# ultralytics/yolov3

Hardware: NVIDIA H100
Metric: images/sec @640 bs32 YOLOv3 (higher is better)
Workload: dtype bf16

## Files before the change

yolov3_b200/csrc/y3_common.cuh:

```cuda
#pragma once
#include <utility>

#include <cuda.h>
#include <cuda_bf16.h>
#include <cuda_fp16.h>
#include <cuda_runtime.h>
#include <stdint.h>

namespace y3 {

#ifndef Y3_WATCHDOG_CYCLES
#define Y3_WATCHDOG_CYCLES 3000000000LL
#endif

__device__ __forceinline__ uint32_t smem_u32(const void* p) {
  return static_cast<uint32_t>(__cvta_generic_to_shared(p));
}

__device__ __forceinline__ void mbar_init(uint64_t* bar, uint32_t count) {
  asm volatile("mbarrier.init.shared::cta.b64 [%0], %1;" ::"r"(smem_u32(bar)), "r"(count) : "memory");
}
__device__ __forceinline__ void fence_mbar_init() {
  asm volatile("fence.mbarrier_init.release.cluster;" ::: "memory");
}
// ... 25 lines not shown
  while (!mbar_try_wait(bar, parity)) {
    if (clock64() - t0 > Y3_WATCHDOG_CYCLES) {
      if (err) atomicExch(err, code);
      __threadfence_system();
      __trap();
    }
  }
}

__device__ __forceinline__ void tma_prefetch_desc(const CUtensorMap* m) {
  asm volatile("prefetch.tensormap [%0];" ::"l"(reinterpret_cast<uint64_t>(m)) : "memory");
}
__device__ __forceinline__ void tma_load_2d(void* dst, const CUtensorMap* m, uint64_t* bar, int c0, int c1) {
  asm volatile(
      "cp.async.bulk.tensor.2d.shared::cluster.global.mbarrier::complete_tx::bytes [%0], [%1, {%3, %4}], [%2];"
      ::"r"(smem_u32(dst)), "l"(reinterpret_cast<uint64_t>(m)), "r"(smem_u32(bar)), "r"(c0), "r"(c1)
      : "memory");
}
__device__ __forceinline__ void tma_load_4d(void* dst, const CUtensorMap* m, uint64_t* bar, int c0, int c1, int c2, int c3) {
  asm volatile(
      "cp.async.bulk.tensor.4d.shared::cluster.global.mbarrier::complete_tx::bytes [%0], [%1, {%3, %4, %5, %6}], [%2];"
      ::"r"(smem_u32(dst)), "l"(reinterpret_cast<uint64_t>(m)), "r"(smem_u32(bar)), "r"(c0), "r"(c1), "r"(c2), "r"(c3)
      : "memory");
}
__device__ __forceinline__ void tma_load_5d(void* dst, const CUtensorMap* m, uint64_t* bar, int c0, int c1, int c2,
                                            int c3, int c4) {
  asm volatile(
      "cp.async.bulk.tensor.5d.shared::cluster.global.mbarrier::complete_tx::bytes [%0], [%1, {%3, %4, %5, %6, %7}], "
      "[%2];"
      ::"r"(smem_u32(dst)), "l"(reinterpret_cast<uint64_t>(m)), "r"(smem_u32(bar)), "r"(c0), "r"(c1), "r"(c2), "r"(c3),
      "r"(c4)
      : "memory");
}

__device__ __forceinline__ void tma_store_2d(const CUtensorMap* m, const void* src, int c0, int c1) {
  asm volatile("cp.async.bulk.tensor.2d.global.shared::cta.bulk_group [%0, {%2, %3}], [%1];" ::"l"(
                   reinterpret_cast<uint64_t>(m)),
               "r"(smem_u32(src)), "r"(c0), "r"(c1)
               : "memory");
}
__device__ __forceinline__ void tma_store_4d(const CUtensorMap* m, const void* src, int c0, int c1, int c2, int c3) {
  asm volatile("cp.async.bulk.tensor.4d.global.shared::cta.bulk_group [%0, {%2, %3, %4, %5}], [%1];" ::"l"(
                   reinterpret_cast<uint64_t>(m)),
               "r"(smem_u32(src)), "r"(c0), "r"(c1), "r"(c2), "r"(c3)
               : "memory");
}
__device__ __forceinline__ void bulk_commit_group() { asm volatile("cp.async.bulk.commit_group;" ::: "memory"); }
__device__ __forceinline__ void bulk_wait_read_all() { asm volatile("cp.async.bulk.wait_group.read 0;" ::: "memory"); }
__device__ __forceinline__ void bulk_wait_read_1() { asm volatile("cp.async.bulk.wait_group.read 1;" ::: "memory"); }
__device__ __forceinline__ void bulk_wait_all() { asm volatile("cp.async.bulk.wait_group 0;" ::: "memory"); }
__device__ __forceinline__ void named_bar_sync(int id, int nthreads) {
  asm volatile("bar.sync %0, %1;" ::"r"(id), "r"(nthreads) : "memory");
}
__device__ __forceinline__ uint4 lds128(uint32_t saddr) {
  uint4 v;
  asm volatile("ld.shared.v4.u32 {%0, %1, %2, %3}, [%4];" : "=r"(v.x), "=r"(v.y), "=r"(v.z), "=r"(v.w) : "r"(saddr));
  return v;
}
__device__ __forceinline__ void sts128(uint32_t saddr, uint4 v) {
  asm volatile("st.shared.v4.u32 [%0], {%1, %2, %3, %4};" ::"r"(saddr), "r"(v.x), "r"(v.y), "r"(v.z), "r"(v.w) : "memory");
}

__device__ __forceinline__ bool elect_one() {
  uint32_t pred;
  asm volatile(
      "{\n"
      ".reg .pred p;\n"
      "elect.sync _|p, 0xffffffff;\n"
      "selp.u32 %0, 1, 0, p;\n"
      "}\n"
      : "=r"(pred));
  return pred != 0;
}

__host__ __device__ constexpr uint32_t wgmma_layout(uint32_t swizzle_bytes) {
  return swizzle_bytes == 128 ? 1u : (swizzle_bytes == 64 ? 2u : 3u);
}
__host__ __device__ constexpr uint32_t wgmma_desc_hi(uint32_t sbo_bytes, uint32_t swizzle_bytes) {
  return ((sbo_bytes >> 4) & 0x3FFFu) | (wgmma_layout(swizzle_bytes) << 30);
}
__device__ __forceinline__ uint64_t wgmma_desc(uint32_t desc_hi, uint32_t saddr, uint32_t lbo_bytes = 0) {
  return (uint64_t(desc_hi) << 32) | ((saddr >> 4) & 0x3FFFu) | (((lbo_bytes >> 4) & 0x3FFFu) << 16);
}
__device__ __forceinline__ void wgmma_fence() { asm volatile("wgmma.fence.sync.aligned;" ::: "memory"); }
__device__ __forceinline__ void wgmma_commit() { asm volatile("wgmma.commit_group.sync.aligned;" ::: "memory"); }
// ... 279 lines not shown
```

yolov3_b200/csrc/y3_conv_tc.cu:

```cuda
#include <cuda_bf16.h>

#include <type_traits>

#include "y3_common.cuh"
#include "y3_internal.h"

namespace y3 {

namespace {

constexpr int kBlockM = 128;
constexpr int kThreads = 320;
constexpr int kProducerWarp = 8;
constexpr int kStoreWarp = 9;
constexpr int kSmemBudget = 221 * 1024;

template <int BLOCK_N, int BLOCK_K, bool HALO, int STAGE_ES = 2, bool STAGE_DQ = false>
struct Cfg {
  static constexpr uint32_t kARows = HALO ? kBlockM + 2 : kBlockM;
  static constexpr uint32_t kATxBytes = kARows * BLOCK_K * 2;
  static constexpr uint32_t kABytes = (kATxBytes + 1023u) / 1024u * 1024u;
  static constexpr uint32_t kTaps = HALO ? 3 : 1;
  static constexpr uint32_t kBBytes = BLOCK_N * BLOCK_K * 2;
  static constexpr uint32_t kStageBytes = kABytes + kTaps * kBBytes;
  static constexpr int kMaxStages = 8;
  static constexpr uint32_t kBarBytes = 256;
  static constexpr bool kStaged = BLOCK_N == 256 && STAGE_ES > 0;
  static constexpr uint32_t kTileBytes = kBlockM * BLOCK_N * (STAGE_ES > 0 ? STAGE_ES : 2);
  static constexpr uint32_t kOutBytes = kTileBytes + BLOCK_N * 4 * (STAGE_DQ ? 2 : 1);
  static constexpr bool kPair = BLOCK_N <= 128 && STAGE_ES > 0;
  static constexpr uint32_t kRowBytes = BLOCK_N * (STAGE_ES > 0 ? STAGE_ES : 2);
  static constexpr uint32_t kBoxBytes = kRowBytes < 128 ? kRowBytes : 128;
  static constexpr uint32_t kBoxes = kRowBytes / kBoxBytes;
  static constexpr uint32_t kPairBytes = 1024 - kBarBytes + 2 * kTileBytes;
  __host__ __device__ static constexpr int ring_stages(uint32_t reserve) {
    const int s = int(kSmemBudget - reserve) / int(kStageBytes);
    return s > kMaxStages ? kMaxStages : s;
  }
  __host__ __device__ static constexpr uint32_t bres_bytes(int steps) { return (uint32_t(steps) * kBBytes + 1023u) / 1024u * 1024u; }
  __host__ __device__ static constexpr int bres_stages(int steps, uint32_t reserve) {
    const int s = (int(kSmemBudget - reserve) - int(bres_bytes(steps))) / int(kABytes);
    return s > kMaxStages ? kMaxStages : s;
  }
  static constexpr uint32_t kSwizzleBytes = BLOCK_K * 2;
  static constexpr uint32_t kSbo = 8 * kSwizzleBytes;
  __host__ __device__ static constexpr uint32_t bar_offset(int stages, bool bres, int b_steps) {
    return uint32_t(stages) * kABytes + (bres ? bres_bytes(b_steps) : uint32_t(stages) * kTaps * kBBytes);
  }
  __host__ __device__ static constexpr uint32_t smem_end(int stages, bool bres, int b_steps, uint32_t reserve) {
    return bar_offset(stages, bres, b_steps) + kBarBytes + reserve;
  }
  static constexpr size_t kSmemBytes = size_t(kSmemBudget) + 1024  + kBarBytes;
  static_assert(ring_stages(kStaged ? kOutBytes : (kPair ? kPairBytes : 0u)) >= 2, "pipeline needs at least two stages");
  static_assert(!HALO || BLOCK_K >= 32, "halo reuse: rows of 64 or 128 bytes");
};

__device__ __forceinline__ float bias_act(float a, float b, bool silu) {
  if (!silu) return a + b;
  const float h = fmaf(a, 0.5f, b);
  float t;
  asm("tanh.approx.f32 %0, %1;" : "=f"(t) : "f"(h));
  return fmaf(h, t, h);
}

__device__ __forceinline__ float bias_act_dq(float a, float s, float b, bool silu) {
  const float h = fmaf(a, s, b);
  if (!silu) return h;
  float t;
  asm("tanh.approx.f32 %0, %1;" : "=f"(t) : "f"(h));
  return fmaf(h, t, h);
}

__device__ __forceinline__ void cp_async16(uint32_t saddr, const void* gptr) {
  asm volatile("cp.async.cg.shared.global [%0], [%1], 16;" ::"r"(saddr), "l"(gptr) : "memory");
}
__device__ __forceinline__ void cp_async_wait_all() { asm volatile("cp.async.wait_all;" ::: "memory"); }

__device__ __forceinline__ uint32_t fast_div(uint32_t n, uint32_t mul, uint32_t shr) {
  const uint32_t t = __umulhi(n, mul);
  return (t + ((n - t) >> (shr ? 1 : 0))) >> (shr ? shr - 1 : 0);
}

struct RowOut {
  __nv_bfloat16* out;
  float* f32;
  const __nv_bfloat16* res;
};

template <int ES, typename T>
__device__ __forceinline__ T* elem_ptr(T* p, long long off) {
  if (ES == 2) return p + off;
  return reinterpret_cast<T*>(reinterpret_cast<uintptr_t>(p) + off * ES);
}

template <int ES = 2>
__device__ __forceinline__ RowOut row_out(const ConvTcArgs& p, int mt, int n0, int m) {
  RowOut o{nullptr, nullptr, nullptr};
  bool valid;
  int img, oy, ox;
  if (p.mode == 0) {
    const int row = mt * kBlockM + m;
    const int plane = p.hp * p.wp;
    img = static_cast<int>(fast_div(static_cast<uint32_t>(row), p.plane_mul, p.plane_shr));
    const int rem = row - img * plane;
    const int yp = static_cast<int>(fast_div(static_cast<uint32_t>(rem), p.wp_mul, p.wp_shr)), xp = rem - yp * p.wp;
    valid = row < p.rows_total && yp >= 1 && yp <= p.hp - 2 && xp >= 1 && xp <= p.wp - 2;
    oy = yp - 1;
    ox = xp - 1;
  } else {
// ... 17 lines not shown
  } else if (p.upsample) {
    const long long r00 = (static_cast<long long>(img) * (2 * oh + 2) + 2 * oy + 1) * (2 * ow + 2) + 2 * ox + 1;
    o.out = elem_ptr<ES>(p.out, r00 * p.out_ld + p.out_coff + n0);
  } else {
    o.out = elem_ptr<ES>(p.out, conv_row * p.out_ld + p.out_coff + n0);
  }
  return o;
}

template <int BLOCK_N, int BLOCK_K, bool HALO, int IN_FMT = Y3_FMT_BF16, int OUT_FMT = Y3_FMT_BF16>
__global__ void __launch_bounds__(kThreads, 1)
conv_tc_kernel(const __grid_constant__ CUtensorMap map_a, const __grid_constant__ CUtensorMap map_b,
               const __grid_constant__ CUtensorMap map_out, const __grid_constant__ CUtensorMap map_res, const ConvTcArgs p) {
  constexpr bool kInE4m3 = IN_FMT == Y3_FMT_E4M3, kOutE4m3 = OUT_FMT == Y3_FMT_E4M3;
  using C = Cfg<BLOCK_N, BLOCK_K, HALO, kOutE4m3 ? 1 : (kInE4m3 ? 0 : 2), kInE4m3 && kOutE4m3>;
  constexpr int kOes = kOutE4m3 ? 1 : 2;
  constexpr int kKch = kInE4m3 ? 2 * BLOCK_K : BLOCK_K;
  using Mma = std::conditional_t<kInE4m3, WgmmaE4m3<BLOCK_N>, Wgmma<BLOCK_N>>;
  const int STAGES = p.stages;
  const bool bres = p.bres != 0;
  constexpr uint32_t kBStage = C::kTaps * C::kBBytes;
  const int b_steps = p.taps * p.kblocks;

  extern __shared__ uint8_t smem_raw[];
  const uint32_t raw_addr = smem_u32(smem_raw);
  uint8_t* smem = smem_raw + ((1024u - (raw_addr & 1023u)) & 1023u);
  uint8_t* smem_a = smem;
  uint8_t* smem_b = smem + STAGES * C::kABytes;
  uint64_t* full_bar = reinterpret_cast<uint64_t*>(smem_b + (bres ? C::bres_bytes(b_steps) : uint32_t(STAGES) * kBStage));
  uint64_t* empty_bar = full_bar + C::kMaxStages;
  uint64_t* bres_bar = empty_bar + C::kMaxStages;
  uint64_t* staged_bar = bres_bar + 1;
  uint64_t* done_bar = bres_bar + 3;
  uint32_t* stile = reinterpret_cast<uint32_t*>(reinterpret_cast<uint8_t*>(full_bar) + C::kBarBytes);
  float* sbias = reinterpret_cast<float*>(stile + C::kTileBytes / 4);
  float* sdq = sbias + BLOCK_N;
  const bool staged_out = C::kStaged && p.out_f32 == nullptr;
  uint8_t* ptile = reinterpret_cast<uint8_t*>(full_bar) + 1024;
  const bool pair_out = C::kPair && p.tile_tma != 0;

  const int warp = threadIdx.x >> 5;
  const int lane = threadIdx.x & 31;

  if (threadIdx.x == 0) {
    tma_prefetch_desc(&map_a);
    tma_prefetch_desc(&map_b);
    if (pair_out) {
      tma_prefetch_desc(&map_out);
      if (p.res) tma_prefetch_desc(&map_res);
    }
    for (int i = 0; i < STAGES; ++i) {
      mbar_init(&full_bar[i], 1);
      mbar_init(&empty_bar[i], 8);
    }
    mbar_init(bres_bar, 1);
    for (int b = 0; b < 2; ++b) {
      mbar_init(&staged_bar[b], pair_out ? 1 : 32);
      mbar_init(&done_bar[b], 8);
    }
    fence_mbar_init();
  }
  __syncthreads();
  pdl_wait();
  pdl_trigger();

  const int total_tiles = p.m_tiles * p.n_tiles;
  const int k_iters = HALO ? 3 * p.kblocks : p.taps * p.kblocks;

  if (warp == kProducerWarp) {
    uint32_t stage = 0, phase = 0;
    if (bres && int(blockIdx.x) < total_tiles && elect_one()) {
      mbar_expect_tx(bres_bar, uint32_t(b_steps) * C::kBBytes);
      for (int st = 0; st < b_steps; ++st) {
        const int kb = st / p.taps, tap = st - kb * p.taps;
        tma_load_2d(smem_b + st * C::kBBytes, &map_b, bres_bar, (p.custom_taps ? p.tap_wcol[tap] : tap) * p.cin + kb * kKch, 0);
      }
    }
    __syncwarp();
    const int n_tiles = p.n_tiles, wp = p.wp, cin = p.cin, a_coff = p.a_coff, a_ld = p.a_ld;
    const int taps_it = HALO ? 3 : p.taps;
    const bool xpair = p.xpair != 0, nine = p.taps == 9, custom = p.custom_taps != 0;
    const int taps_w = xpair ? 2 : 3;
    const uint32_t stage_tx = p.a_tx_bytes + (bres ? 0u : kBStage);
    auto run = [&](auto mode_tag) {
      constexpr int MODE = decltype(mode_tag)::value;
      for (int tile = blockIdx.x; tile < total_tiles; tile += gridDim.x) {
        const int nt = tile % n_tiles;
        const int mt = tile / n_tiles;
        const int n0 = nt * BLOCK_N;
        int row0 = 0, img = 0, oh0 = 0, ow0 = 0;
// ... 21 lines not shown
            if (MODE == 0)
              tma_load_2d(a_dst, &map_a, &full_bar[stage], a_coff + kcol, row0 + shift);
            else
              tma_load_5d(a_dst, &map_a, &full_bar[stage], c0, ow0 + c1, r & 1, oh0 + (r >> 1), img);
            if (!bres) {
#pragma unroll
              for (uint32_t t = 0; t < C::kTaps; ++t)
                tma_load_2d(b_dst + t * C::kBBytes, &map_b, &full_bar[stage], bcol + int(t) * cin, n0);
            }
          }
          __syncwarp();
          if (++stage == uint32_t(STAGES)) {
            stage = 0;
            phase ^= 1u;
          }
          if (++s == taps_w) {
            s = 0;
            ++r;
          }
          if (++tap == taps_it) {
            tap = 0;
            r = 0;
            s = 0;
            ++kb;
          }
        }
      }
    };
    if (p.mode == 0)
      run(std::integral_constant<int, 0>{});
    else
      run(std::integral_constant<int, 1>{});
  } else if (warp == kStoreWarp) {
    if (pair_out) {
      if (lane != 0) return;
      const uint32_t res_tx = uint32_t(p.mode == 0 ? kBlockM : p.tw * p.th) * C::kRowBytes;
      constexpr int kBoxCh = C::kBoxBytes / kOes;
      auto move = [&](int tile, int b, bool load) {
        const int mt = tile / p.n_tiles, n0 = (tile % p.n_tiles) * BLOCK_N;
        int c1 = mt * kBlockM, c2 = 0, c3 = 0;
        if (p.mode != 0) {
          const int per_img = p.tiles_w * p.tiles_h;
          c3 = mt / per_img;
          const int t = mt - c3 * per_img;
          c1 = (t % p.tiles_w) * p.tw;
          c2 = (t / p.tiles_w) * p.th;
        }
#pragma unroll
        for (uint32_t k = 0; k < C::kBoxes; ++k) {
          uint8_t* s = ptile + b * C::kTileBytes + k * kBlockM * C::kBoxBytes;
          const int c0 = (load ? p.res_coff : p.out_coff) + n0 + int(k) * kBoxCh;
          if (load) {
            if (p.mode == 0) tma_load_2d(s, &map_res, &staged_bar[b], c0, c1);
            else tma_load_4d(s, &map_res, &staged_bar[b], c0, c1, c2, c3);
          } else {
            if (p.mode == 0) tma_store_2d(&map_out, s, c0, c1);
            else tma_store_4d(&map_out, s, c0, c1, c2, c3);
          }
        }
      };
      auto stage = [&](int tile, int b) {
        if (p.res) {
          mbar_expect_tx(&staged_bar[b], res_tx);
          move(tile, b, true);
        } else {
          mbar_arrive(&staged_bar[b]);
        }
      };
      const int step = int(gridDim.x);
      if (int(blockIdx.x) < total_tiles) stage(blockIdx.x, 0);
      if (int(blockIdx.x) + step < total_tiles) stage(blockIdx.x + step, 1);
      for (int tile = blockIdx.x, i = 0; tile < total_tiles; tile += step, ++i) {
        const int b = i & 1;
        mbar_wait(&done_bar[b], uint32_t(i >> 1) & 1u, p.err, 9);
        move(tile, b, false);
        bulk_commit_group();
        if (tile + 2 * step < total_tiles) {
          bulk_wait_read_all();
          stage(tile + 2 * step, b);
        }
      }
      bulk_wait_all();
      return;
    }
    if (!staged_out) return;
    const int r = lane & 7, c = lane >> 3;
    const uint32_t stile_s = smem_u32(stile);
    struct Rows {
      __nv_bfloat16* out[4];
      const __nv_bfloat16* res[4];
    };
    auto rows_of = [&](int tile, Rows& R) {
      const int mt = tile / p.n_tiles, n0 = (tile % p.n_tiles) * BLOCK_N;
#pragma unroll
      for (int q = 0; q < 4; ++q) {
        const RowOut ro = row_out<kOes>(p, mt, n0, 32 * q + lane);
        R.out[q] = ro.out;
        R.res[q] = ro.res;
      }
    };
    constexpr int kCh = 16 / kOes, kRowChunks = BLOCK_N / kCh;
    auto chunk = [&](int h, int w, int j) { return uint32_t((h * kRowChunks + j) * 64 + w * 8 + r); };
    auto src_lane = [&](int h, int w) { return (w & 1) * 16 + 8 * h + r; };
    auto stage_bias = [&](int tile) {
      const int n0 = (tile % p.n_tiles) * BLOCK_N;
      for (int i = lane; i < BLOCK_N / 4; i += 32)
        if (n0 + 4 * i < p.cout) {
          cp_async16(smem_u32(sbias + 4 * i), p.bias + n0 + 4 * i);
          if (kInE4m3) cp_async16(smem_u32(sdq + 4 * i), p.dq + n0 + 4 * i);
        }
    };
    auto stage_res = [&](int tile, const Rows& R) {
      const int n0 = (tile % p.n_tiles) * BLOCK_N;
      if (p.res) {
#pragma unroll
        for (int h = 0; h < 2; ++h)
#pragma unroll
          for (int w = 0; w < 8; ++w) {
            const auto* res = reinterpret_cast<const __nv_bfloat16*>(
                __shfl_sync(~0u, reinterpret_cast<unsigned long long>(R.res[2 * (w >> 2) + ((w & 3) >> 1)]), src_lane(h, w)));
            if (!res) continue;
#pragma unroll 1
            for (int jg = 0; jg < kRowChunks / 4; ++jg) {
              const int j = 4 * jg + c;
              if (kOutE4m3 ? n0 + kCh * j < p.cout : n0 + 32 * jg < p.cout)
                cp_async16(stile_s + 16u * chunk(h, w, j), elem_ptr<kOes>(res, kCh * j));
            }
          }
      }
      cp_async_wait_all();
      mbar_arrive(staged_bar);
    };
    auto drain = [&](int tile, const Rows& R) {
      const int n0 = (tile % p.n_tiles) * BLOCK_N;
      const long long up_row_stride = static_cast<long long>(2 * (p.mode == 0 ? p.wp - 2 : p.wo) + 2) * p.out_ld;
      const int reps = p.upsample ? 4 : 1;
      const uint4* tile16 = reinterpret_cast<const uint4*>(stile);
#pragma unroll
      for (int h = 0; h < 2; ++h)
#pragma unroll
        for (int w = 0; w < 8; ++w) {
          auto* out = reinterpret_cast<__nv_bfloat16*>(
              __shfl_sync(~0u, reinterpret_cast<unsigned long long>(R.out[2 * (w >> 2) + ((w & 3) >> 1)]), src_lane(h, w)));
          if (!out) continue;
#pragma unroll 2
          for (int jg = 0; jg < kRowChunks / 4; ++jg) {
            const int j = 4 * jg + c;
            if (kOutE4m3 ? n0 + kCh * j >= p.cout : n0 + 32 * jg >= p.cout) break;
            const uint4 v = tile16[chunk(h, w, j)];
            for (int rep = 0; rep < reps; ++rep)
              *reinterpret_cast<uint4*>(elem_ptr<kOes>(out, (rep >> 1) * up_row_stride + (rep & 1) * p.out_ld + kCh * j)) = v;
          }
        }
    };
    uint32_t tphase = 0;
    Rows cur, nxt;
    if (int(blockIdx.x) < total_tiles) {
      rows_of(blockIdx.x, cur);
      stage_bias(blockIdx.x);
      stage_res(blockIdx.x, cur);
    }
    for (int tile = blockIdx.x; tile < total_tiles; tile += gridDim.x) {
      const int next = tile + int(gridDim.x);
      if (next < total_tiles) rows_of(next, nxt);
      mbar_wait(done_bar, tphase, p.err, 7);
      tphase ^= 1u;
      if (next < total_tiles) stage_bias(next);
      drain(tile, cur);
      if (next < total_tiles) stage_res(next, nxt);
      cur = nxt;
    }
  } else {
    const int wg = warp >> 2;
    const int m0 = wg * 64 + (warp & 3) * 16 + (lane >> 2);
    const int cq = 2 * (lane & 3);
    constexpr uint32_t kDescHi = wgmma_desc_hi(C::kSbo, C::kSwizzleBytes);
    const uint32_t a_base = smem_u32(smem_a) + uint32_t(wg) * 64u * C::kSwizzleBytes;
    const uint32_t b_base = smem_u32(smem_b);
    uint32_t stage = 0, phase = 0, tphase = 0;
    if (bres && int(blockIdx.x) < total_tiles) mbar_wait(bres_bar, 0, p.err, 6);
    for (int tile = blockIdx.x, ti = 0; tile < total_tiles; tile += gridDim.x, ++ti) {
      float acc[BLOCK_N / 2];
      uint32_t prev = 0;
      for (int it = 0; it < k_iters; ++it) {
        mbar_wait(&full_bar[stage], phase, p.err, 3);
        const uint32_t a_st = a_base + stage * C::kABytes;
        const uint32_t b_st = b_base + (bres ? uint32_t(it) : stage) * kBStage;
        wgmma_fence();
#pragma unroll
        for (uint32_t t = 0; t < C::kTaps; ++t) {
#pragma unroll
          for (int k = 0; k < BLOCK_K / 16; ++k) {
            const uint64_t adesc = wgmma_desc(kDescHi, a_st + t * C::kSwizzleBytes + k * 32);
            const uint64_t bdesc = wgmma_desc(kDescHi, b_st + t * C::kBBytes + k * 32);
            Mma::template mma<0, 0>(acc, adesc, bdesc, (it != 0 || t != 0 || k != 0) ? 1u : 0u);
          }
        }
        wgmma_commit();
        wgmma_wait<1>();
        if (it > 0 && lane == 0) mbar_arrive(&empty_bar[prev]);
        prev = stage;
        if (++stage == uint32_t(STAGES)) {
          stage = 0;
          phase ^= 1u;
        }
      }
      wgmma_wait<0>();
      wgmma_fence_regs(acc);
      if (lane == 0) mbar_arrive(&empty_bar[prev]);

      const bool silu = p.act == Y3_ACT_SILU;
      const float bscale = silu ? 0.5f : 1.0f;
      if (staged_out) {
        mbar_wait(staged_bar, tphase, p.err, 8);
        tphase ^= 1u;
        const bool has_res = p.res != nullptr;
        if constexpr (kOutE4m3) {
          uint8_t* tb = reinterpret_cast<uint8_t*>(stile) + ((warp * 8 + (lane >> 2)) * 16 + cq);
#pragma unroll
          for (int j = 0; j < BLOCK_N / 8; ++j) {
            const float2 b = *reinterpret_cast<const float2*>(sbias + 8 * j + cq);
            float2 q = b;
            if (kInE4m3) q = *reinterpret_cast<const float2*>(sdq + 8 * j + cq);
#pragma unroll
            for (int h = 0; h < 2; ++h) {
              uint16_t& hw = *reinterpret_cast<uint16_t*>(tb + (h * BLOCK_N / 16 + j / 2) * 64 * 16 + (j & 1) * 8);
              float x0, x1;
              if (kInE4m3) {
                x0 = bias_act_dq(acc[4 * j + 2 * h], bscale * q.x, bscale * b.x, silu);
                x1 = bias_act_dq(acc[4 * j + 2 * h + 1], bscale * q.y, bscale * b.y, silu);
              } else {
                x0 = bias_act(acc[4 * j + 2 * h], bscale * b.x, silu);
                x1 = bias_act(acc[4 * j + 2 * h + 1], bscale * b.y, silu);
              }
              if (has_res) {
                const float2 f = unpack_e4m3x2(hw);
                x0 = fmaf(p.res_scale, f.x, x0);
                x1 = fmaf(p.res_scale, f.y, x1);
              }
              hw = pack_e4m3x2(x0 * p.out_inv_scale, x1 * p.out_inv_scale);
            }
          }
          __syncwarp();
          if (lane == 0) mbar_arrive(done_bar);
          continue;
        }
        uint32_t* words = stile + threadIdx.x;
#pragma unroll
        for (int j = 0; j < BLOCK_N / 8; ++j) {
          const float2 b = *reinterpret_cast<const float2*>(sbias + 8 * j + cq);
#pragma unroll
          for (int h = 0; h < 2; ++h) {
            uint32_t& word = words[(h * BLOCK_N / 8 + j) * 256];
            float x0 = bias_act(acc[4 * j + 2 * h], bscale * b.x, silu);
            float x1 = bias_act(acc[4 * j + 2 * h + 1], bscale * b.y, silu);
            if (has_res) {
              const float2 f = unpack_bf16x2(word);
              x0 += f.x;
              x1 += f.y;
            }
            word = pack_bf16x2(x0, x1);
          }
        }
        __syncwarp();
        if (lane == 0) mbar_arrive(done_bar);
      } else if (pair_out) {
        const int b = ti & 1;
        mbar_wait(&staged_bar[b], uint32_t(ti >> 1) & 1u, p.err, 10);
        uint8_t* tb = ptile + b * C::kTileBytes;
        const int n0 = (tile % p.n_tiles) * BLOCK_N;
        const bool has_res = p.res != nullptr;
        uint32_t rowoff[2], sw[2];
        bool valid[2];
#pragma unroll
        for (int h = 0; h < 2; ++h) {
          const int m = m0 + 8 * h;
          rowoff[h] = uint32_t(m) * C::kBoxBytes;
          sw[h] = ((rowoff[h] >> 7) & (C::kBoxBytes / 16 - 1)) << 4;
          valid[h] = true;
          if (p.mode == 0) {
            const int row = (tile / p.n_tiles) * kBlockM + m;
            const int img = static_cast<int>(fast_div(static_cast<uint32_t>(row), p.plane_mul, p.plane_shr));
            const int rem = row - img * (p.hp * p.wp);
            const int yp = static_cast<int>(fast_div(static_cast<uint32_t>(rem), p.wp_mul, p.wp_shr)), xp = rem - yp * p.wp;
            valid[h] = yp >= 1 && yp <= p.hp - 2 && xp >= 1 && xp <= p.wp - 2;
          }
        }
#pragma unroll
        for (int j = 0; j < BLOCK_N / 8; ++j) {
          const int c = 8 * j + cq;
          const bool in = n0 + c < p.cout;
          const float2 bv = in ? __ldg(reinterpret_cast<const float2*>(p.bias + n0 + c)) : make_float2(0.f, 0.f);
          float2 qv = bv;
          if (kInE4m3) qv = in ? __ldg(reinterpret_cast<const float2*>(p.dq + n0 + c)) : make_float2(0.f, 0.f);
          const uint32_t xb = uint32_t(8 * j * kOes);
          const uint32_t region = xb / C::kBoxBytes * (kBlockM * C::kBoxBytes), xin = xb % C::kBoxBytes;
#pragma unroll
          for (int h = 0; h < 2; ++h) {
            uint8_t* pp = tb + region + rowoff[h] + (xin ^ sw[h]) + cq * kOes;
            float x0, x1;
            if (kInE4m3) {
              x0 = bias_act_dq(acc[4 * j + 2 * h], bscale * qv.x, bscale * bv.x, silu);
              x1 = bias_act_dq(acc[4 * j + 2 * h + 1], bscale * qv.y, bscale * bv.y, silu);
            } else {
              x0 = bias_act(acc[4 * j + 2 * h], bscale * bv.x, silu);
              x1 = bias_act(acc[4 * j + 2 * h + 1], bscale * bv.y, silu);
            }
            if constexpr (kOutE4m3) {
              uint16_t& hw = *reinterpret_cast<uint16_t*>(pp);
              if (has_res) {
                const float2 f = unpack_e4m3x2(hw);
                x0 = fmaf(p.res_scale, f.x, x0);
                x1 = fmaf(p.res_scale, f.y, x1);
              }
              hw = valid[h] ? pack_e4m3x2(x0 * p.out_inv_scale, x1 * p.out_inv_scale) : uint16_t(0);
            } else {
              uint32_t& word = *reinterpret_cast<uint32_t*>(pp);
              if (has_res) {
                const float2 f = unpack_bf16x2(word);
                x0 += f.x;
                x1 += f.y;
              }
              word = valid[h] ? pack_bf16x2(x0, x1) : 0u;
            }
          }
        }
        fence_proxy_async_smem();
        __syncwarp();
        if (lane == 0) mbar_arrive(&done_bar[b]);
      } else {
        const int mt = tile / p.n_tiles, n0 = (tile % p.n_tiles) * BLOCK_N;
        const long long up_row_stride = static_cast<long long>(2 * (p.mode == 0 ? p.wp - 2 : p.wo) + 2) * p.out_ld;
        const int reps = p.upsample ? 4 : 1;
        constexpr int kChunk = BLOCK_N == 256 ? 1 : (kInE4m3 && BLOCK_N == 128 ? 8 : (BLOCK_N / 8 < 16 ? BLOCK_N / 8 : 16));
#pragma unroll
        for (int h = 0; h < 2; ++h) {
          const RowOut ro = row_out<kOes>(p, mt, n0, m0 + 8 * h);
          if (!ro.f32 && !ro.out) continue;
#pragma unroll
          for (int j0 = 0; j0 < BLOCK_N / 8; j0 += kChunk) {
            float2 b[kChunk], q[kChunk];
            uint32_t r[kChunk];
#pragma unroll
            for (int jj = 0; jj < kChunk; ++jj) {
              const int c = 8 * (j0 + jj) + cq;
              const bool in = p.out_f32 || n0 + c < p.cout;
              b[jj] = in ? __ldg(reinterpret_cast<const float2*>(p.bias + n0 + c)) : make_float2(0.f, 0.f);
              if (kInE4m3) q[jj] = in ? __ldg(reinterpret_cast<const float2*>(p.dq + n0 + c)) : make_float2(0.f, 0.f);
              if (kOutE4m3)
                r[jj] = (in && ro.res) ? __ldcg(reinterpret_cast<const unsigned short*>(elem_ptr<1>(ro.res, c))) : 0u;
              else
                r[jj] = (in && ro.res) ? __ldcg(reinterpret_cast<const unsigned int*>(ro.res + c)) : 0u;
            }
#pragma unroll
            for (int jj = 0; jj < kChunk; ++jj) {
              const int c = 8 * (j0 + jj) + cq;
              if (!p.out_f32 && n0 + c >= p.cout) continue;
              float x0, x1;
              if (kInE4m3) {
                x0 = bias_act_dq(acc[4 * (j0 + jj) + 2 * h], bscale * q[jj].x, bscale * b[jj].x, silu);
                x1 = bias_act_dq(acc[4 * (j0 + jj) + 2 * h + 1], bscale * q[jj].y, bscale * b[jj].y, silu);
              } else {
                x0 = bias_act(acc[4 * (j0 + jj) + 2 * h], bscale * b[jj].x, silu);
                x1 = bias_act(acc[4 * (j0 + jj) + 2 * h + 1], bscale * b[jj].y, silu);
              }
              if (ro.f32) {
                *reinterpret_cast<float2*>(ro.f32 + c) = make_float2(x0, x1);
              } else if (kOutE4m3) {
                if (ro.res) {
                  const float2 f = unpack_e4m3x2(static_cast<uint16_t>(r[jj]));
                  x0 = fmaf(p.res_scale, f.x, x0);
// ... 1 lines not shown
                }
                const uint16_t v = pack_e4m3x2(x0 * p.out_inv_scale, x1 * p.out_inv_scale);
                for (int rep = 0; rep < reps; ++rep)
                  *reinterpret_cast<uint16_t*>(elem_ptr<1>(ro.out, (rep >> 1) * up_row_stride + (rep & 1) * p.out_ld + c)) = v;
              } else {
                if (ro.res) {
                  const float2 f = unpack_bf16x2(r[jj]);
                  x0 += f.x;
                  x1 += f.y;
                }
                const uint32_t v = pack_bf16x2(x0, x1);
                for (int rep = 0; rep < reps; ++rep)
                  *reinterpret_cast<uint32_t*>(ro.out + (rep >> 1) * up_row_stride + (rep & 1) * p.out_ld + c) = v;
              }
            }
          }
        }
      }
    }
  }
}

template <int BLOCK_N, int BLOCK_K, bool HALO = false, int IN_FMT = Y3_FMT_BF16, int OUT_FMT = Y3_FMT_BF16>
int launch_cfg(const ConvTcPlan& plan, cudaStream_t stream) {
  constexpr bool kInE4m3 = IN_FMT == Y3_FMT_E4M3, kOutE4m3 = OUT_FMT == Y3_FMT_E4M3;
  using C = Cfg<BLOCK_N, BLOCK_K, HALO, kOutE4m3 ? 1 : (kInE4m3 ? 0 : 2), kInE4m3 && kOutE4m3>;
  auto kern = conv_tc_kernel<BLOCK_N, BLOCK_K, HALO, IN_FMT, OUT_FMT>;
  static bool attr_set = false;
  if (!attr_set) {
    Y3_CHECK_CUDA(cudaFuncSetAttribute(kern, cudaFuncAttributeMaxDynamicSharedMemorySize, int(C::kSmemBytes)));
    attr_set = true;
  }
  ConvTcArgs args = plan.args;
  const bool out_tile = C::kStaged && args.out_f32 == nullptr;
  const bool pair = C::kPair && args.tile_tma != 0;
  const uint32_t reserve = out_tile ? C::kOutBytes : (pair ? C::kPairBytes : 0u);
  const int b_steps = args.taps * args.kblocks;
  args.bres = plan.bres;
  args.stages = plan.bres ? C::bres_stages(b_steps, reserve) : C::ring_stages(reserve);
  if (args.bres && args.stages < 3) {
    args.bres = 0;
    args.stages = C::ring_stages(reserve);
  }
  if (args.stages < 2 || args.stages > C::kMaxStages ||
      C::smem_end(args.stages, args.bres != 0, b_steps, reserve) + 1024u > C::kSmemBytes)
    return set_error(Y3_ERR_BAD_ARG, "conv_tc: %d ring stages (resident weights %d, output tiles %u bytes) do not fit %zu bytes of shared memory (N=%d K=%d)",
                     args.stages, args.bres, reserve, C::kSmemBytes, BLOCK_N, BLOCK_K);
  Y3_CHECK_CUDA(launch_pdl(kern, dim3(plan.grid), dim3(kThreads), C::kSmemBytes, stream, plan.map_a, plan.map_b,
                           plan.map_out, plan.map_res, args));
  return Y3_OK;
}

int pick_block_n(int cout) { return cout <= 32 ? 32 : (cout <= 64 ? 64 : (cout <= 128 ? 128 : 256)); }

template <int IN_FMT, int OUT_FMT>
int launch_fmt(const ConvTcPlan& plan, cudaStream_t stream) {
#define Y3_DISPATCH_K(BN)                                                        \
  switch (plan.block_k) {                                                        \
    case 64: return launch_cfg<BN, 64, false, IN_FMT, OUT_FMT>(plan, stream);    \
    case 32: return launch_cfg<BN, 32, false, IN_FMT, OUT_FMT>(plan, stream);    \
    case 16: return launch_cfg<BN, 16, false, IN_FMT, OUT_FMT>(plan, stream);    \
  }                                                                              \
  break;
  constexpr bool kHalo = !(IN_FMT == Y3_FMT_E4M3 && OUT_FMT == Y3_FMT_BF16);
  if (plan.halo) {
    if constexpr (kHalo) {
      if (plan.block_k == 64) {
        if (plan.block_n == 128) return launch_cfg<128, 64, true, IN_FMT, OUT_FMT>(plan, stream);
        if (plan.block_n == 64) return launch_cfg<64, 64, true, IN_FMT, OUT_FMT>(plan, stream);
// ... 177 lines not shown
      const int thc = th > a.ho ? a.ho : th;
      const long long tiles = static_cast<long long>((a.wo + tw - 1) / tw) * ((a.ho + thc - 1) / thc);
      if (best_tiles < 0 || tiles < best_tiles || (tiles == best_tiles && tw > best_tw)) {
        best_tiles = tiles;
        best_tw = tw;
        best_th = thc;
      }
    }
    a.tw = best_tw;
    a.th = best_th;
    a.tiles_w = (a.wo + a.tw - 1) / a.tw;
    a.tiles_h = (a.ho + a.th - 1) / a.th;
    a.m_tiles = d.n * a.tiles_w * a.tiles_h;
    a.a_tx_bytes = static_cast<uint32_t>(a.tw) * a.th * bk * 2;
    const uint64_t ld = static_cast<uint64_t>(d.in_ld);
    const uint64_t dims[5] = {2 * ld, static_cast<uint64_t>(wp / 2), 2, static_cast<uint64_t>(hp / 2),
                              static_cast<uint64_t>(d.n)};
    const uint64_t strides[5] = {0, 2 * ld * es, static_cast<uint64_t>(wp) * ld * es, 2ull * wp * ld * es,
                                 static_cast<uint64_t>(hp) * wp * ld * es};
    const uint32_t box[5] = {static_cast<uint32_t>(kch), static_cast<uint32_t>(a.tw), 1, static_cast<uint32_t>(a.th), 1};
    rc = select_only ? Y3_OK : encode_tensor_map(&plan->map_a, d.in_fmt, d.in, 5, dims, strides, box, bk * 2);
    if (rc) return rc;
  }
  {
    const uint64_t ktot = static_cast<uint64_t>(extra ? d.ksize * d.ksize : taps) * gemm_cin;
    const uint64_t dims[2] = {ktot, static_cast<uint64_t>(cout_pad)};
    const uint64_t strides[2] = {0, ktot * es};
    const uint32_t box[2] = {static_cast<uint32_t>(kch), static_cast<uint32_t>(bn)};
    rc = select_only ? Y3_OK : encode_tensor_map(&plan->map_b, d.in_fmt, d.weight, 2, dims, strides, box, bk * 2);
    if (rc) return rc;
  }
  plan->map_out = CUtensorMap{};
  plan->map_res = CUtensorMap{};
  a.tile_tma = (!head && bn <= 128 && !d.upsample && !(extra && extra->phase)) ? 1 : 0;
  if (a.tile_tma && !select_only) {
    const int oes = out8 ? 1 : 2;
    const int box_bytes = bn * oes < 128 ? bn * oes : 128;
    const uint32_t box_ch = static_cast<uint32_t>(box_bytes / oes);
    auto encode_out = [&](CUtensorMap* m, const void* base, int ld, int coff) {
      const uint64_t pitch = static_cast<uint64_t>(ld) * oes;
      if (a.mode == 0) {
        const uint64_t dims[2] = {static_cast<uint64_t>(coff + d.c_out), static_cast<uint64_t>(a.rows_total)};
        const uint64_t strides[2] = {0, pitch};
        const uint32_t box[2] = {box_ch, kBlockM};
        return encode_tensor_map(m, plan->out_fmt, base, 2, dims, strides, box, box_bytes);
      }
      const uint64_t wpo = static_cast<uint64_t>(a.wo) + 2, hpo = static_cast<uint64_t>(a.ho) + 2;
      const void* interior = static_cast<const uint8_t*>(base) + (wpo + 1) * pitch;
      const uint64_t dims[4] = {static_cast<uint64_t>(coff + d.c_out), static_cast<uint64_t>(a.wo),
                                static_cast<uint64_t>(a.ho), static_cast<uint64_t>(d.n)};
      const uint64_t strides[4] = {0, pitch, wpo * pitch, hpo * wpo * pitch};
      const uint32_t box[4] = {box_ch, static_cast<uint32_t>(a.tw), static_cast<uint32_t>(a.th), 1};
      return encode_tensor_map(m, plan->out_fmt, interior, 4, dims, strides, box, box_bytes);
    };
    rc = encode_out(&plan->map_out, d.out, d.out_ld, d.out_coff);
    if (rc) return rc;
    if (d.res) {
      rc = encode_out(&plan->map_res, d.res, d.res_ld, d.res_coff);
      if (rc) return rc;
    }
  }
  {
    const long long b_bytes = static_cast<long long>(taps) * a.kblocks * bn * bk * 2;
    plan->bres = (a.n_tiles == 1 && b_bytes <= 96 * 1024) ? 1 : 0;
  }
  const int sms = num_sms();
  const long long total = static_cast<long long>(a.m_tiles) * a.n_tiles;
// ... 73 lines not shown
```

Baseline: 1800.

## Unify conv epilogue on TMA tile stores, including BLOCK_N=256 with bulk-loaded bias

Drops the separate BLOCK_N=256 staged-output path, where a store warp copied tiles to global with per-lane 16-byte stores and cp.async. Every tile size now goes through the TMA tile store/residual-load path, with one or two buffers depending on tile size. For 256-wide tiles the bias and dequant scales are bulk-loaded into shared memory on the same mbarrier as the residual. Large tiles get only one buffer, so the epilogue overlaps less with the next tile's compute, and smem addressing is rewritten with explicit swizzled lds/sts.

```diff
diff --git a/yolov3_b200/csrc/y3_common.cuh b/yolov3_b200/csrc/y3_common.cuh
--- a/yolov3_b200/csrc/y3_common.cuh
+++ b/yolov3_b200/csrc/y3_common.cuh
@@ -81,6 +81,11 @@
       "r"(c4)
       : "memory");
 }
+__device__ __forceinline__ void bulk_load(void* dst, const void* src, uint32_t bytes, uint64_t* bar) {
+  asm volatile("cp.async.bulk.shared::cluster.global.mbarrier::complete_tx::bytes [%0], [%1], %2, [%3];"
+               ::"r"(smem_u32(dst)), "l"(reinterpret_cast<uint64_t>(src)), "r"(bytes), "r"(smem_u32(bar))
+               : "memory");
+}
 
 __device__ __forceinline__ void tma_store_2d(const CUtensorMap* m, const void* src, int c0, int c1) {
   asm volatile("cp.async.bulk.tensor.2d.global.shared::cta.bulk_group [%0, {%2, %3}], [%1];" ::"l"(
@@ -100,6 +105,27 @@
 __device__ __forceinline__ void bulk_wait_all() { asm volatile("cp.async.bulk.wait_group 0;" ::: "memory"); }
 __device__ __forceinline__ void named_bar_sync(int id, int nthreads) {
   asm volatile("bar.sync %0, %1;" ::"r"(id), "r"(nthreads) : "memory");
+}
+__device__ __forceinline__ uint32_t lds32(uint32_t saddr) {
+  uint32_t v;
+  asm volatile("ld.shared.b32 %0, [%1];" : "=r"(v) : "r"(saddr));
+  return v;
+}
+__device__ __forceinline__ void sts32(uint32_t saddr, uint32_t v) {
+  asm volatile("st.shared.b32 [%0], %1;" ::"r"(saddr), "r"(v) : "memory");
+}
+__device__ __forceinline__ float2 lds_f32x2(uint32_t saddr) {
+  float2 v;
+  asm volatile("ld.shared.v2.f32 {%0, %1}, [%2];" : "=f"(v.x), "=f"(v.y) : "r"(saddr));
+  return v;
+}
+__device__ __forceinline__ uint16_t lds16(uint32_t saddr) {
+  uint16_t v;
+  asm volatile("ld.shared.b16 %0, [%1];" : "=h"(v) : "r"(saddr));
+  return v;
+}
+__device__ __forceinline__ void sts16(uint32_t saddr, uint16_t v) {
+  asm volatile("st.shared.b16 [%0], %1;" ::"r"(saddr), "h"(v) : "memory");
 }
 __device__ __forceinline__ uint4 lds128(uint32_t saddr) {
   uint4 v;
diff --git a/yolov3_b200/csrc/y3_conv_tc.cu b/yolov3_b200/csrc/y3_conv_tc.cu
--- a/yolov3_b200/csrc/y3_conv_tc.cu
+++ b/yolov3_b200/csrc/y3_conv_tc.cu
@@ -25,14 +25,14 @@
   static constexpr uint32_t kStageBytes = kABytes + kTaps * kBBytes;
   static constexpr int kMaxStages = 8;
   static constexpr uint32_t kBarBytes = 256;
-  static constexpr bool kStaged = BLOCK_N == 256 && STAGE_ES > 0;
-  static constexpr uint32_t kTileBytes = kBlockM * BLOCK_N * (STAGE_ES > 0 ? STAGE_ES : 2);
-  static constexpr uint32_t kOutBytes = kTileBytes + BLOCK_N * 4 * (STAGE_DQ ? 2 : 1);
-  static constexpr bool kPair = BLOCK_N <= 128 && STAGE_ES > 0;
   static constexpr uint32_t kRowBytes = BLOCK_N * (STAGE_ES > 0 ? STAGE_ES : 2);
+  static constexpr uint32_t kTileBytes = kBlockM * kRowBytes;
   static constexpr uint32_t kBoxBytes = kRowBytes < 128 ? kRowBytes : 128;
   static constexpr uint32_t kBoxes = kRowBytes / kBoxBytes;
-  static constexpr uint32_t kPairBytes = 1024 - kBarBytes + 2 * kTileBytes;
+  static constexpr int kBufs = STAGE_ES == 0 ? 0 : (kTileBytes > 32 * 1024 ? 1 : 2);
+  static constexpr bool kSBias = BLOCK_N == 256 && kBufs > 0;
+  static constexpr uint32_t kBiasBytes = kSBias ? BLOCK_N * 4 * (STAGE_DQ ? 2 : 1) : 0;
+  static constexpr uint32_t kTileReserve = 1024 - kBarBytes + kBufs * (kTileBytes + kBiasBytes);
   __host__ __device__ static constexpr int ring_stages(uint32_t reserve) {
     const int s = int(kSmemBudget - reserve) / int(kStageBytes);
     return s > kMaxStages ? kMaxStages : s;
@@ -51,7 +51,7 @@
     return bar_offset(stages, bres, b_steps) + kBarBytes + reserve;
   }
   static constexpr size_t kSmemBytes = size_t(kSmemBudget) + 1024  + kBarBytes;
-  static_assert(ring_stages(kStaged ? kOutBytes : (kPair ? kPairBytes : 0u)) >= 2, "pipeline needs at least two stages");
+  static_assert(ring_stages(kTileReserve) >= 2, "pipeline needs at least two stages");
   static_assert(!HALO || BLOCK_K >= 32, "halo reuse: rows of 64 or 128 bytes");
 };
 
@@ -70,11 +70,6 @@
   asm("tanh.approx.f32 %0, %1;" : "=f"(t) : "f"(h));
   return fmaf(h, t, h);
 }
-
-__device__ __forceinline__ void cp_async16(uint32_t saddr, const void* gptr) {
-  asm volatile("cp.async.cg.shared.global [%0], [%1], 16;" ::"r"(saddr), "l"(gptr) : "memory");
-}
-__device__ __forceinline__ void cp_async_wait_all() { asm volatile("cp.async.wait_all;" ::: "memory"); }
 
 __device__ __forceinline__ uint32_t fast_div(uint32_t n, uint32_t mul, uint32_t shr) {
   const uint32_t t = __umulhi(n, mul);
@@ -158,12 +153,9 @@
   uint64_t* bres_bar = empty_bar + C::kMaxStages;
   uint64_t* staged_bar = bres_bar + 1;
   uint64_t* done_bar = bres_bar + 3;
-  uint32_t* stile = reinterpret_cast<uint32_t*>(reinterpret_cast<uint8_t*>(full_bar) + C::kBarBytes);
-  float* sbias = reinterpret_cast<float*>(stile + C::kTileBytes / 4);
-  float* sdq = sbias + BLOCK_N;
-  const bool staged_out = C::kStaged && p.out_f32 == nullptr;
-  uint8_t* ptile = reinterpret_cast<uint8_t*>(full_bar) + 1024;
-  const bool pair_out = C::kPair && p.tile_tma != 0;
+  uint8_t* otile = reinterpret_cast<uint8_t*>(full_bar) + 1024;
+  const bool tile_out = C::kBufs > 0 && p.tile_tma != 0;
+  constexpr int kBufs = C::kBufs > 0 ? C::kBufs : 1;
 
   const int warp = threadIdx.x >> 5;
   const int lane = threadIdx.x & 31;
@@ -171,7 +163,7 @@
   if (threadIdx.x == 0) {
     tma_prefetch_desc(&map_a);
     tma_prefetch_desc(&map_b);
-    if (pair_out) {
+    if (tile_out) {
       tma_prefetch_desc(&map_out);
       if (p.res) tma_prefetch_desc(&map_res);
     }
@@ -181,7 +173,7 @@
     }
     mbar_init(bres_bar, 1);
     for (int b = 0; b < 2; ++b) {
-      mbar_init(&staged_bar[b], pair_out ? 1 : 32);
+      mbar_init(&staged_bar[b], 1);
       mbar_init(&done_bar[b], 8);
     }
     fence_mbar_init();
@@ -269,7 +261,7 @@
     else
       run(std::integral_constant<int, 1>{});
   } else if (warp == kStoreWarp) {
-    if (pair_out) {
+    if (tile_out) {
       if (lane != 0) return;
       const uint32_t res_tx = uint32_t(p.mode == 0 ? kBlockM : p.tw * p.th) * C::kRowBytes;
       constexpr int kBoxCh = C::kBoxBytes / kOes;
@@ -285,7 +277,7 @@
         }
 #pragma unroll
         for (uint32_t k = 0; k < C::kBoxes; ++k) {
-          uint8_t* s = ptile + b * C::kTileBytes + k * kBlockM * C::kBoxBytes;
+          uint8_t* s = otile + b * C::kTileBytes + k * kBlockM * C::kBoxBytes;
           const int c0 = (load ? p.res_coff : p.out_coff) + n0 + int(k) * kBoxCh;
           if (load) {
             if (p.mode == 0) tma_load_2d(s, &map_res, &staged_bar[b], c0, c1);
@@ -297,115 +289,36 @@
         }
       };
       auto stage = [&](int tile, int b) {
-        if (p.res) {
-          mbar_expect_tx(&staged_bar[b], res_tx);
-          move(tile, b, true);
-        } else {
+        const int n0 = (tile % p.n_tiles) * BLOCK_N;
+        const uint32_t bias_tx = C::kSBias ? uint32_t(min(BLOCK_N, p.cout - n0)) * 4u : 0u;
+        const uint32_t tx = (p.res ? res_tx : 0u) + bias_tx * (kInE4m3 ? 2u : 1u);
+        if (tx == 0) {
           mbar_arrive(&staged_bar[b]);
+          return;
+        }
+        mbar_expect_tx(&staged_bar[b], tx);
+        if (p.res) move(tile, b, true);
+        if constexpr (C::kSBias) {
+          uint8_t* sb = otile + C::kBufs * C::kTileBytes + b * C::kBiasBytes;
+          bulk_load(sb, p.bias + n0, bias_tx, &staged_bar[b]);
+          if (kInE4m3) bulk_load(sb + BLOCK_N * 4, p.dq + n0, bias_tx, &staged_bar[b]);
         }
       };
       const int step = int(gridDim.x);
-      if (int(blockIdx.x) < total_tiles) stage(blockIdx.x, 0);
-      if (int(blockIdx.x) + step < total_tiles) stage(blockIdx.x + step, 1);
+#pragma unroll
+      for (int i = 0; i < kBufs; ++i)
+        if (int(blockIdx.x) + i * step < total_tiles) stage(blockIdx.x + i * step, i);
       for (int tile = blockIdx.x, i = 0; tile < total_tiles; tile += step, ++i) {
-        const int b = i & 1;
-        mbar_wait(&done_bar[b], uint32_t(i >> 1) & 1u, p.err, 9);
+        const int b = i % kBufs;
+        mbar_wait(&done_bar[b], uint32_t(i / kBufs) & 1u, p.err, 9);
         move(tile, b, false);
         bulk_commit_group();
-        if (tile + 2 * step < total_tiles) {
+        if (tile + kBufs * step < total_tiles) {
           bulk_wait_read_all();
-          stage(tile + 2 * step, b);
+          stage(tile + kBufs * step, b);
         }
       }
       bulk_wait_all();
-      return;
-    }
-    if (!staged_out) return;
-    const int r = lane & 7, c = lane >> 3;
-    const uint32_t stile_s = smem_u32(stile);
-    struct Rows {
-      __nv_bfloat16* out[4];
-      const __nv_bfloat16* res[4];
-    };
-    auto rows_of = [&](int tile, Rows& R) {
-      const int mt = tile / p.n_tiles, n0 = (tile % p.n_tiles) * BLOCK_N;
-#pragma unroll
-      for (int q = 0; q < 4; ++q) {
-        const RowOut ro = row_out<kOes>(p, mt, n0, 32 * q + lane);
-        R.out[q] = ro.out;
-        R.res[q] = ro.res;
-      }
-    };
-    constexpr int kCh = 16 / kOes, kRowChunks = BLOCK_N / kCh;
-    auto chunk = [&](int h, int w, int j) { return uint32_t((h * kRowChunks + j) * 64 + w * 8 + r); };
-    auto src_lane = [&](int h, int w) { return (w & 1) * 16 + 8 * h + r; };
-    auto stage_bias = [&](int tile) {
-      const int n0 = (tile % p.n_tiles) * BLOCK_N;
-      for (int i = lane; i < BLOCK_N / 4; i += 32)
-        if (n0 + 4 * i < p.cout) {
-          cp_async16(smem_u32(sbias + 4 * i), p.bias + n0 + 4 * i);
-          if (kInE4m3) cp_async16(smem_u32(sdq + 4 * i), p.dq + n0 + 4 * i);
-        }
-    };
-    auto stage_res = [&](int tile, const Rows& R) {
-      const int n0 = (tile % p.n_tiles) * BLOCK_N;
-      if (p.res) {
-#pragma unroll
-        for (int h = 0; h < 2; ++h)
-#pragma unroll
-          for (int w = 0; w < 8; ++w) {
-            const auto* res = reinterpret_cast<const __nv_bfloat16*>(
-                __shfl_sync(~0u, reinterpret_cast<unsigned long long>(R.res[2 * (w >> 2) + ((w & 3) >> 1)]), src_lane(h, w)));
-            if (!res) continue;
-#pragma unroll 1
-            for (int jg = 0; jg < kRowChunks / 4; ++jg) {
-              const int j = 4 * jg + c;
-              if (kOutE4m3 ? n0 + kCh * j < p.cout : n0 + 32 * jg < p.cout)
-                cp_async16(stile_s + 16u * chunk(h, w, j), elem_ptr<kOes>(res, kCh * j));
-            }
-          }
-      }
-      cp_async_wait_all();
-      mbar_arrive(staged_bar);
-    };
-    auto drain = [&](int tile, const Rows& R) {
-      const int n0 = (tile % p.n_tiles) * BLOCK_N;
-      const long long up_row_stride = static_cast<long long>(2 * (p.mode == 0 ? p.wp - 2 : p.wo) + 2) * p.out_ld;
-      const int reps = p.upsample ? 4 : 1;
-      const uint4* tile16 = reinterpret_cast<const uint4*>(stile);
-#pragma unroll
-      for (int h = 0; h < 2; ++h)
-#pragma unroll
-        for (int w = 0; w < 8; ++w) {
-          auto* out = reinterpret_cast<__nv_bfloat16*>(
-              __shfl_sync(~0u, reinterpret_cast<unsigned long long>(R.out[2 * (w >> 2) + ((w & 3) >> 1)]), src_lane(h, w)));
-          if (!out) continue;
-#pragma unroll 2
-          for (int jg = 0; jg < kRowChunks / 4; ++jg) {
-            const int j = 4 * jg + c;
-            if (kOutE4m3 ? n0 + kCh * j >= p.cout : n0 + 32 * jg >= p.cout) break;
-            const uint4 v = tile16[chunk(h, w, j)];
-            for (int rep = 0; rep < reps; ++rep)
-              *reinterpret_cast<uint4*>(elem_ptr<kOes>(out, (rep >> 1) * up_row_stride + (rep & 1) * p.out_ld + kCh * j)) = v;
-          }
-        }
-    };
-    uint32_t tphase = 0;
-    Rows cur, nxt;
-    if (int(blockIdx.x) < total_tiles) {
-      rows_of(blockIdx.x, cur);
-      stage_bias(blockIdx.x);
-      stage_res(blockIdx.x, cur);
-    }
-    for (int tile = blockIdx.x; tile < total_tiles; tile += gridDim.x) {
-      const int next = tile + int(gridDim.x);
-      if (next < total_tiles) rows_of(next, nxt);
-      mbar_wait(done_bar, tphase, p.err, 7);
-      tphase ^= 1u;
-      if (next < total_tiles) stage_bias(next);
-      drain(tile, cur);
-      if (next < total_tiles) stage_res(next, nxt);
-      cur = nxt;
     }
   } else {
     const int wg = warp >> 2;
@@ -414,9 +327,9 @@
     constexpr uint32_t kDescHi = wgmma_desc_hi(C::kSbo, C::kSwizzleBytes);
     const uint32_t a_base = smem_u32(smem_a) + uint32_t(wg) * 64u * C::kSwizzleBytes;
     const uint32_t b_base = smem_u32(smem_b);
-    uint32_t stage = 0, phase = 0, tphase = 0;
+    uint32_t stage = 0, phase = 0;
     if (bres && int(blockIdx.x) < total_tiles) mbar_wait(bres_bar, 0, p.err, 6);
-    for (int tile = blockIdx.x, ti = 0; tile < total_tiles; tile += gridDim.x, ++ti) {
+    for (int tile = blockIdx.x; tile < total_tiles; tile += gridDim.x) {
       float acc[BLOCK_N / 2];
       uint32_t prev = 0;
       for (int it = 0; it < k_iters; ++it) {
@@ -448,75 +361,20 @@
 
       const bool silu = p.act == Y3_ACT_SILU;
       const float bscale = silu ? 0.5f : 1.0f;
-      if (staged_out) {
-        mbar_wait(staged_bar, tphase, p.err, 8);
-        tphase ^= 1u;
-        const bool has_res = p.res != nullptr;
-        if constexpr (kOutE4m3) {
-          uint8_t* tb = reinterpret_cast<uint8_t*>(stile) + ((warp * 8 + (lane >> 2)) * 16 + cq);
-#pragma unroll
-          for (int j = 0; j < BLOCK_N / 8; ++j) {
-            const float2 b = *reinterpret_cast<const float2*>(sbias + 8 * j + cq);
-            float2 q = b;
-            if (kInE4m3) q = *reinterpret_cast<const float2*>(sdq + 8 * j + cq);
-#pragma unroll
-            for (int h = 0; h < 2; ++h) {
-              uint16_t& hw = *reinterpret_cast<uint16_t*>(tb + (h * BLOCK_N / 16 + j / 2) * 64 * 16 + (j & 1) * 8);
-              float x0, x1;
-              if (kInE4m3) {
-                x0 = bias_act_dq(acc[4 * j + 2 * h], bscale * q.x, bscale * b.x, silu);
-                x1 = bias_act_dq(acc[4 * j + 2 * h + 1], bscale * q.y, bscale * b.y, silu);
-              } else {
-                x0 = bias_act(acc[4 * j + 2 * h], bscale * b.x, silu);
-                x1 = bias_act(acc[4 * j + 2 * h + 1], bscale * b.y, silu);
-              }
-              if (has_res) {
-                const float2 f = unpack_e4m3x2(hw);
-                x0 = fmaf(p.res_scale, f.x, x0);
-                x1 = fmaf(p.res_scale, f.y, x1);
-              }
-              hw = pack_e4m3x2(x0 * p.out_inv_scale, x1 * p.out_inv_scale);
-            }
-          }
-          __syncwarp();
-          if (lane == 0) mbar_arrive(done_bar);
-          continue;
-        }
-        uint32_t* words = stile + threadIdx.x;
-#pragma unroll
-        for (int j = 0; j < BLOCK_N / 8; ++j) {
-          const float2 b = *reinterpret_cast<const float2*>(sbias + 8 * j + cq);
-#pragma unroll
-          for (int h = 0; h < 2; ++h) {
-            uint32_t& word = words[(h * BLOCK_N / 8 + j) * 256];
-            float x0 = bias_act(acc[4 * j + 2 * h], bscale * b.x, silu);
-            float x1 = bias_act(acc[4 * j + 2 * h + 1], bscale * b.y, silu);
-            if (has_res) {
-              const float2 f = unpack_bf16x2(word);
-              x0 += f.x;
-              x1 += f.y;
-            }
-            word = pack_bf16x2(x0, x1);
-          }
-        }
-        __syncwarp();
-        if (lane == 0) mbar_arrive(done_bar);
-      } else if (pair_out) {
-        const int b = ti & 1;
-        mbar_wait(&staged_bar[b], uint32_t(ti >> 1) & 1u, p.err, 10);
-        uint8_t* tb = ptile + b * C::kTileBytes;
+      if (tile_out) {
+        const int ti = (tile - int(blockIdx.x)) / int(gridDim.x);
+        const int b = ti % kBufs;
+        mbar_wait(&staged_bar[b], uint32_t(ti / kBufs) & 1u, p.err, 10);
         const int n0 = (tile % p.n_tiles) * BLOCK_N;
         const bool has_res = p.res != nullptr;
-        uint32_t rowoff[2], sw[2];
-        bool valid[2];
-#pragma unroll
-        for (int h = 0; h < 2; ++h) {
-          const int m = m0 + 8 * h;
-          rowoff[h] = uint32_t(m) * C::kBoxBytes;
-          sw[h] = ((rowoff[h] >> 7) & (C::kBoxBytes / 16 - 1)) << 4;
-          valid[h] = true;
-          if (p.mode == 0) {
-            const int row = (tile / p.n_tiles) * kBlockM + m;
+        const uint32_t sw = ((uint32_t(m0) * C::kBoxBytes >> 7) & (C::kBoxBytes / 16 - 1)) << 4;
+        const uint32_t row_s = ((smem_u32(otile) + uint32_t(m0) * C::kBoxBytes + cq * kOes) ^ sw) + b * C::kTileBytes;
+        const uint32_t bias_s = smem_u32(otile) + C::kBufs * C::kTileBytes + b * C::kBiasBytes + cq * 4;
+        bool valid[2] = {true, true};
+        if (p.mode == 0) {
+#pragma unroll
+          for (int h = 0; h < 2; ++h) {
+            const int row = (tile / p.n_tiles) * kBlockM + m0 + 8 * h;
             const int img = static_cast<int>(fast_div(static_cast<uint32_t>(row), p.plane_mul, p.plane_shr));
             const int rem = row - img * (p.hp * p.wp);
             const int yp = static_cast<int>(fast_div(static_cast<uint32_t>(rem), p.wp_mul, p.wp_shr)), xp = rem - yp * p.wp;
@@ -526,15 +384,21 @@
 #pragma unroll
         for (int j = 0; j < BLOCK_N / 8; ++j) {
           const int c = 8 * j + cq;
-          const bool in = n0 + c < p.cout;
-          const float2 bv = in ? __ldg(reinterpret_cast<const float2*>(p.bias + n0 + c)) : make_float2(0.f, 0.f);
-          float2 qv = bv;
-          if (kInE4m3) qv = in ? __ldg(reinterpret_cast<const float2*>(p.dq + n0 + c)) : make_float2(0.f, 0.f);
+          float2 bv, qv;
+          if constexpr (C::kSBias) {
+            bv = lds_f32x2(bias_s + 32 * j);
+            qv = kInE4m3 ? lds_f32x2(bias_s + 4 * BLOCK_N + 32 * j) : bv;
+          } else {
+            const bool in = n0 + c < p.cout;
+            bv = in ? __ldg(reinterpret_cast<const float2*>(p.bias + n0 + c)) : make_float2(0.f, 0.f);
+            qv = bv;
+            if (kInE4m3) qv = in ? __ldg(reinterpret_cast<const float2*>(p.dq + n0 + c)) : make_float2(0.f, 0.f);
+          }
           const uint32_t xb = uint32_t(8 * j * kOes);
           const uint32_t region = xb / C::kBoxBytes * (kBlockM * C::kBoxBytes), xin = xb % C::kBoxBytes;
 #pragma unroll
           for (int h = 0; h < 2; ++h) {
-            uint8_t* pp = tb + region + rowoff[h] + (xin ^ sw[h]) + cq * kOes;
+            const uint32_t pp = (row_s ^ xin) + region + 8 * h * C::kBoxBytes;
             float x0, x1;
             if (kInE4m3) {
               x0 = bias_act_dq(acc[4 * j + 2 * h], bscale * qv.x, bscale * bv.x, silu);
@@ -544,21 +408,19 @@
               x1 = bias_act(acc[4 * j + 2 * h + 1], bscale * bv.y, silu);
             }
             if constexpr (kOutE4m3) {
-              uint16_t& hw = *reinterpret_cast<uint16_t*>(pp);
               if (has_res) {
-                const float2 f = unpack_e4m3x2(hw);
+                const float2 f = unpack_e4m3x2(lds16(pp));
                 x0 = fmaf(p.res_scale, f.x, x0);
                 x1 = fmaf(p.res_scale, f.y, x1);
               }
-              hw = valid[h] ? pack_e4m3x2(x0 * p.out_inv_scale, x1 * p.out_inv_scale) : uint16_t(0);
+              sts16(pp, valid[h] ? pack_e4m3x2(x0 * p.out_inv_scale, x1 * p.out_inv_scale) : uint16_t(0));
             } else {
-              uint32_t& word = *reinterpret_cast<uint32_t*>(pp);
               if (has_res) {
-                const float2 f = unpack_bf16x2(word);
+                const float2 f = unpack_bf16x2(lds32(pp));
                 x0 += f.x;
                 x1 += f.y;
               }
-              word = valid[h] ? pack_bf16x2(x0, x1) : 0u;
+              sts32(pp, valid[h] ? pack_bf16x2(x0, x1) : 0u);
             }
           }
         }
@@ -567,13 +429,13 @@
         if (lane == 0) mbar_arrive(&done_bar[b]);
       } else {
         const int mt = tile / p.n_tiles, n0 = (tile % p.n_tiles) * BLOCK_N;
-        const long long up_row_stride = static_cast<long long>(2 * (p.mode == 0 ? p.wp - 2 : p.wo) + 2) * p.out_ld;
-        const int reps = p.upsample ? 4 : 1;
         constexpr int kChunk = BLOCK_N == 256 ? 1 : (kInE4m3 && BLOCK_N == 128 ? 8 : (BLOCK_N / 8 < 16 ? BLOCK_N / 8 : 16));
 #pragma unroll
         for (int h = 0; h < 2; ++h) {
           const RowOut ro = row_out<kOes>(p, mt, n0, m0 + 8 * h);
           if (!ro.f32 && !ro.out) continue;
+          const long long up_row_stride = static_cast<long long>(2 * (p.mode == 0 ? p.wp - 2 : p.wo) + 2) * p.out_ld;
+          const int reps = p.upsample ? 4 : 1;
 #pragma unroll
           for (int j0 = 0; j0 < BLOCK_N / 8; j0 += kChunk) {
             float2 b[kChunk], q[kChunk];
@@ -641,9 +503,7 @@
     attr_set = true;
   }
   ConvTcArgs args = plan.args;
-  const bool out_tile = C::kStaged && args.out_f32 == nullptr;
-  const bool pair = C::kPair && args.tile_tma != 0;
-  const uint32_t reserve = out_tile ? C::kOutBytes : (pair ? C::kPairBytes : 0u);
+  const uint32_t reserve = (C::kBufs > 0 && args.tile_tma != 0) ? C::kTileReserve : 0u;
   const int b_steps = args.taps * args.kblocks;
   args.bres = plan.bres;
   args.stages = plan.bres ? C::bres_stages(b_steps, reserve) : C::ring_stages(reserve);
@@ -887,7 +747,7 @@
   }
   plan->map_out = CUtensorMap{};
   plan->map_res = CUtensorMap{};
-  a.tile_tma = (!head && bn <= 128 && !d.upsample && !(extra && extra->phase)) ? 1 : 0;
+  a.tile_tma = (!head && !d.upsample && !(extra && extra->phase)) ? 1 : 0;
   if (a.tile_tma && !select_only) {
     const int oes = out8 ? 1 : 2;
     const int box_bytes = bn * oes < 128 ? bn * oes : 128;
```

After: 2085, median of 6. +15.8%, better.
